# JzHuai0108/sim3opt

Measured on AMD Instinct MI355X. Metric: LM iterations/s, higher is better.
Workload: dtype f64

## Files before the change

sim3opt_amd/csrc/lm_kernels.hpp:

```cpp
#pragma once
__global__ __launch_bounds__(WG) void k_final_sum(const double* __restrict__ partials, int n,
                                                  double* __restrict__ out) {
  __shared__ double sh[4];
  const double s = sum_partials(partials, n, sh);
  if (threadIdx.x == 0) *out = s;
}

__global__ __launch_bounds__(WG) void k_final_trace_max(const double* __restrict__ trace_partials,
                                                        const double* __restrict__ max_partials, int n,
                                                        double* __restrict__ trace_out,
                                                        unsigned long long* __restrict__ maxdiag_bits) {
  __shared__ double sh[4];
  __shared__ double shm[4];
  const double s = sum_partials(trace_partials, n, sh);
  double m = 0.0;
  for (int i = threadIdx.x; i < n; i += WG) m = fmax(m, max_partials[i]);
#pragma unroll
  for (int off = 32; off > 0; off >>= 1) m = fmax(m, __shfl_xor(m, off));
  if ((threadIdx.x & 63) == 0) shm[threadIdx.x >> 6] = m;
  __syncthreads();
  if (threadIdx.x == 0) {
    *trace_out = s;
    m = fmax(fmax(shm[0], shm[1]), fmax(shm[2], shm[3]));
    *maxdiag_bits = (unsigned long long)__double_as_longlong(m);
  }
}

__global__ __launch_bounds__(WG) void k_final_sum_two(const double* __restrict__ pa, int na,
                                                      double* __restrict__ outa,
                                                      const double* __restrict__ pb, int nb_,
                                                      double* __restrict__ outb,
                                                      DevScalars* __restrict__ host_mirror,
                                                      const DevScalars* __restrict__ dev_sc) {
  __shared__ double sh[4];
  const double a = sum_partials(pa, na, sh);
  const double b = sum_partials(pb, nb_, sh);
  if (threadIdx.x == 0) {
    *outa = a;
    *outb = b;
    if (host_mirror) {
      host_mirror->chi2 = a;
      host_mirror->scale = b;
      host_mirror->fail = dev_sc->fail;
    }
  }
}

__device__ __forceinline__ double quad_form(const double e[7], const double* __restrict__ Om) {
  double acc = 0.0;
#pragma unroll
  for (int c = 0; c < 7; ++c) {
    double col = 0.0;
#pragma unroll
    for (int r = 0; r < 7; ++r) col += e[r] * Om[7 * c + r];
    acc += col * e[c];
  }
  return acc;
}

__device__ __forceinline__ void huber(double e2, double delta, double& rho, double& w) {
  const double dsqr = delta * delta;
  if (e2 <= dsqr) {
    rho = e2;
    w = 1.0;
  } else {
    const double sq = sqrt(e2);
    rho = 2 * sq * delta - dsqr;
    w = delta / sq;
  }
}


struct EdgeArgs {
  int32_t e_lo, e_hi;
  const int32_t* ev0;
  const int32_t* ev1;
  const Sim3* meas;
  const double* info;
  const double* kdelta;
  const Sim3* states;
  sim3::Opts opts;
};

__global__ __launch_bounds__(WG) void k_chi2(EdgeArgs A, double* __restrict__ partials) {
  __shared__ double sh[4];
  double acc = 0.0;
  for (int k = A.e_lo + blockIdx.x * WG + threadIdx.x; k < A.e_hi; k += gridDim.x * WG) {
    const Sim3 C = load_sim3(A.meas + k);
    const Sim3 S0 = load_sim3(A.states + A.ev0[k]);
    const Sim3 S1 = load_sim3(A.states + A.ev1[k]);
    double e[7];
    sim3::edge_error(C, S0, S1, A.opts, e);
    double chi;
    if (A.info) {
      chi = quad_form(e, A.info + (size_t)49 * k);
    } else {
      chi = 0.0;
#pragma unroll
      for (int r = 0; r < 7; ++r) chi += e[r] * e[r];
    }
    if (A.kdelta && A.kdelta[k] > 0.0) {
      double rho, w;
      huber(chi, A.kdelta[k], rho, w);
      chi = rho;
    }
    acc += chi;
  }
  const double s = block_sum(acc, sh);
  if (threadIdx.x == 0) partials[blockIdx.x] = s;
}

__global__ __launch_bounds__(WG) void k_edge_errors(EdgeArgs A, double* __restrict__ out) {
  for (int k = A.e_lo + blockIdx.x * WG + threadIdx.x; k < A.e_hi; k += gridDim.x * WG) {
    const Sim3 C = load_sim3(A.meas + k);
    const Sim3 S0 = load_sim3(A.states + A.ev0[k]);
    const Sim3 S1 = load_sim3(A.states + A.ev1[k]);
    double e[7];
    sim3::edge_error(C, S0, S1, A.opts, e);
#pragma unroll
    for (int r = 0; r < 7; ++r) out[(size_t)7 * k + r] = e[r];
  }
}

struct LinArgs {
  int32_t n_active;
  const int32_t* active;
  const int32_t* ev0;
  const int32_t* ev1;
  const Sim3* meas;
  const double* info;
  const double* kdelta;
  const Sim3* states;
  const int32_t* slot01;
  const int32_t* slot10;
  const int32_t* inc0;
  const int32_t* inc1;
  double* vals;
  double* scratch;
  double delta;
  sim3::Opts opts;
  const Sim3* ptab;
  int32_t dof_mask;
  DevScalars* sc;
};

struct GramTables {
  unsigned char ga[119], gb[119];
  unsigned char tr[28], tc[28];
};
__constant__ GramTables c_tab;

constexpr int EPB = 8;

__global__ __launch_bounds__(64) void k_perturbation_table(double delta, sim3::Opts opts, Sim3* __restrict__ tab) {
  const int t = threadIdx.x;
  if (t >= 14) return;
  const int d = t >> 1;
  const double step = (t & 1) ? -delta : delta;
  double xi[7];
#pragma unroll
  for (int i = 0; i < 7; ++i) xi[i] = (i == d) ? step : 0.0;
  tab[t] = sim3::exp(xi, opts);
}

template <bool HAS_INFO, bool HAS_KERNEL>
__device__ __forceinline__ void linearize_gram_store(const LinArgs& A, int edge, bool valid, int l,
                                                     double (*J)[7], double (*O)[7], double (*G)[15]) {
  __syncthreads();
  if (HAS_INFO) {
    if (valid) {
      const double* Om = A.info + (size_t)49 * edge;
      for (int t = l; t < 105; t += 32) {
        const int a = t / 7, r = t % 7;
        double acc = 0.0;
#pragma unroll
        for (int k = 0; k < 7; ++k) acc += Om[7 * k + r] * J[a][k];
        O[a][r] = acc;
      }
    }
    __syncthreads();
  }
  double (*OJ)[7] = HAS_INFO ? O : J;
  double w = 1.0;
  if (HAS_KERNEL) {
    if (valid && A.kdelta[edge] > 0.0) {
      double chi = 0.0, rho;
#pragma unroll
      for (int r = 0; r < 7; ++r) chi += J[14][r] * OJ[14][r];
      huber(chi, A.kdelta[edge], rho, w);
    }
  }
  if (valid) {
    for (int t = l; t < 119; t += 32) {
      const int a = c_tab.ga[t], b = c_tab.gb[t];
      double acc = 0.0;
#pragma unroll
      for (int r = 0; r < 7; ++r) acc += J[a][r] * OJ[b][r];
      G[a][b] = (b == 14 ? -w : w) * acc;
    }
  }
  __syncthreads();
  if (valid) {
    const int s01 = A.slot01[edge], s10 = A.slot10[edge];
    const int i0 = A.inc0[edge], i1 = A.inc1[edge];
    for (int o = l; o < 168; o += 32) {
      if (o < 49) {
        if (s01 >= 0) A.vals[(size_t)49 * s01 + o] = G[o % 7][7 + o / 7];
      } else if (o < 98) {
        const int p = o - 49;
        if (s10 >= 0) A.vals[(size_t)49 * s10 + p] = G[p / 7][7 + p % 7];
      } else if (o < 133) {
        const int t = o - 98;
        if (i0 >= 0)
          A.scratch[(size_t)35 * i0 + t] = t < 28 ? G[c_tab.tr[t]][c_tab.tc[t]] : G[t - 28][14];
      } else {
        const int t = o - 133;
        if (i1 >= 0)
          A.scratch[(size_t)35 * i1 + t] =
              t < 28 ? G[7 + c_tab.tr[t]][7 + c_tab.tc[t]] : G[7 + t - 28][14];
      }
    }
  }
}

template <bool HAS_INFO, bool HAS_KERNEL>
__global__ __launch_bounds__(WG) void k_linearize_numeric(LinArgs A) {
  __shared__ double s_in[EPB][24];
  __shared__ double s_J[EPB][15][7];
  __shared__ double s_O[HAS_INFO ? EPB : 1][15][7];
  __shared__ double s_G[EPB][14][15];
  const int l = threadIdx.x & 31, es = threadIdx.x >> 5;
  const int ai = blockIdx.x * EPB + es;
  const bool valid = ai < A.n_active;
  if (blockIdx.x == 0 && threadIdx.x == 0) A.sc->maxdiag_bits = 0ull;
  int edge = 0;
  if (valid) {
    edge = A.active[ai];
    if (l < 8) s_in[es][l] = reinterpret_cast<const double*>(A.meas + edge)[l];
    else if (l < 16) s_in[es][l] = reinterpret_cast<const double*>(A.states + A.ev0[edge])[l - 8];
    else if (l < 24) s_in[es][l] = reinterpret_cast<const double*>(A.states + A.ev1[edge])[l - 16];
  }
  __syncthreads();
  double e[7] = {0, 0, 0, 0, 0, 0, 0};
  if (valid && l < 29) {
    Sim3 C, S0, S1;
    const double* in = s_in[es];
    C.q[0] = in[0]; C.q[1] = in[1]; C.q[2] = in[2]; C.q[3] = in[3];
    C.t[0] = in[4]; C.t[1] = in[5]; C.t[2] = in[6]; C.s = in[7];
    S0.q[0] = in[8]; S0.q[1] = in[9]; S0.q[2] = in[10]; S0.q[3] = in[11];
    S0.t[0] = in[12]; S0.t[1] = in[13]; S0.t[2] = in[14]; S0.s = in[15];
    S1.q[0] = in[16]; S1.q[1] = in[17]; S1.q[2] = in[18]; S1.q[3] = in[19];
    S1.t[0] = in[20]; S1.t[1] = in[21]; S1.t[2] = in[22]; S1.s = in[23];
    if (l < 28) {
      const Sim3 P = A.ptab[l % 14];
      if (l < 14) S0 = sim3::mul(P, S0);
      else S1 = sim3::mul(P, S1);
    }
    sim3::edge_error(C, S0, S1, A.opts, e);
  }
  const double scalar = 1.0 / (2.0 * A.delta);
#pragma unroll
  for (int r = 0; r < 7; ++r) {
    const double other = __shfl_down(e[r], 1);
    if (valid && l < 28 && !(l & 1))
      s_J[es][l >> 1][r] = ((A.dof_mask >> ((l % 14) >> 1)) & 1) ? scalar * (e[r] - other) : 0.0;
    if (valid && l == 28) s_J[es][14][r] = e[r];
  }
  linearize_gram_store<HAS_INFO, HAS_KERNEL>(A, edge, valid, l, s_J[es], HAS_INFO ? s_O[es] : s_J[es], s_G[es]);
}

template <bool HAS_INFO, bool HAS_KERNEL>
__global__ __launch_bounds__(WG) void k_linearize_analytic(LinArgs A) {
  constexpr int NJ = EPB * 15 * 7, NO = HAS_INFO ? NJ : 7, NG = EPB * 14 * 15;
  constexpr int NS = sim3::JAC_SUMS + 13;
  constexpr int NN = EPB * (sim3::JAC_NODES + 1) * sim3::JAC_SUMS, NM = EPB * NS;
  constexpr int NLDS = NN + NM > NJ + NO + NG ? NN + NM : NJ + NO + NG;
  __shared__ double s_in[EPB][24];
  __shared__ double s_lds[NLDS];
  double (*s_node)[sim3::JAC_NODES + 1][sim3::JAC_SUMS] =
      reinterpret_cast<double (*)[sim3::JAC_NODES + 1][sim3::JAC_SUMS]>(s_lds);
  double (*s_M)[NS] = reinterpret_cast<double (*)[NS]>(s_lds + NN);
  double (*s_J)[15][7] = reinterpret_cast<double (*)[15][7]>(s_lds);
  double (*s_O)[15][7] = reinterpret_cast<double (*)[15][7]>(s_lds + NJ);
  double (*s_G)[14][15] = reinterpret_cast<double (*)[14][15]>(s_lds + NJ + NO);
  const int l = threadIdx.x & 31, es = threadIdx.x >> 5;
  const int ai = blockIdx.x * EPB + es;
  const bool valid = ai < A.n_active;
  if (blockIdx.x == 0 && threadIdx.x == 0) A.sc->maxdiag_bits = 0ull;
  int edge = 0;
  if (valid) {
    edge = A.active[ai];
    if (l < 8) s_in[es][l] = reinterpret_cast<const double*>(A.meas + edge)[l];
    else if (l < 16) s_in[es][l] = reinterpret_cast<const double*>(A.states + A.ev0[edge])[l - 8];
    else if (l < 24) s_in[es][l] = reinterpret_cast<const double*>(A.states + A.ev1[edge])[l - 16];
  }
  __syncthreads();
  double e[7] = {0, 0, 0, 0, 0, 0, 0};
  Sim3 C;
  if (valid) {
    Sim3 S0, S1;
    const double* in = s_in[es];
    C.q[0] = in[0]; C.q[1] = in[1]; C.q[2] = in[2]; C.q[3] = in[3];
    C.t[0] = in[4]; C.t[1] = in[5]; C.t[2] = in[6]; C.s = in[7];
    S0.q[0] = in[8]; S0.q[1] = in[9]; S0.q[2] = in[10]; S0.q[3] = in[11];
    S0.t[0] = in[12]; S0.t[1] = in[13]; S0.t[2] = in[14]; S0.s = in[15];
    S1.q[0] = in[16]; S1.q[1] = in[17]; S1.q[2] = in[18]; S1.q[3] = in[19];
    S1.t[0] = in[20]; S1.t[1] = in[21]; S1.t[2] = in[22]; S1.s = in[23];
    sim3::edge_error(C, S0, S1, A.opts, e);
    if (l < sim3::JAC_NODES) {
      double v[sim3::JAC_SUMS];
      sim3::left_jacobian_node(e, l, v);
#pragma unroll
      for (int i = 0; i < sim3::JAC_SUMS; ++i) s_node[es][l][i] = v[i];
    } else if (l == sim3::JAC_NODES) {
      double X[13];
      sim3::exp_of_residual(e, X);
#pragma unroll
      for (int i = 0; i < 13; ++i) s_node[es][l][i] = X[i];
    }
  }
  __syncthreads();
  if (valid && l < sim3::JAC_SUMS) {
    double acc = 0.0;
#pragma unroll
    for (int k = 0; k < sim3::JAC_NODES; ++k) acc += s_node[es][k][l];
    s_M[es][l] = acc;
    if (l < 13) s_M[es][sim3::JAC_SUMS + l] = s_node[es][sim3::JAC_NODES][l];
  }
  __syncthreads();
  if (valid && l < 15) {
    double col[7];
    if (l < 14) {
      sim3::edge_jacobian_column(s_M[es], s_M[es] + sim3::JAC_SUMS, C, l, A.dof_mask, col);
    } else {
#pragma unroll
      for (int r = 0; r < 7; ++r) col[r] = e[r];
    }
#pragma unroll
    for (int r = 0; r < 7; ++r) s_J[es][l][r] = col[r];
  }
  linearize_gram_store<HAS_INFO, HAS_KERNEL>(A, edge, valid, l, s_J[es], HAS_INFO ? s_O[es] : s_J[es], s_G[es]);
}

__global__ __launch_bounds__(WG) void k_edge_jacobians(EdgeArgs A, int dof_mask, double* __restrict__ e_out,
                                                      double* __restrict__ J_out) {
  for (int k = A.e_lo + blockIdx.x * WG + threadIdx.x; k < A.e_hi; k += gridDim.x * WG) {
    const Sim3 C = load_sim3(A.meas + k);
    const Sim3 S0 = load_sim3(A.states + A.ev0[k]);
    const Sim3 S1 = load_sim3(A.states + A.ev1[k]);
    double e[7], M[sim3::JAC_SUMS], X[13];
    sim3::edge_error(C, S0, S1, A.opts, e);
    sim3::left_jacobian_blocks(e, M);
    sim3::exp_of_residual(e, X);
#pragma unroll
    for (int r = 0; r < 7; ++r) e_out[(size_t)7 * k + r] = e[r];
    for (int c = 0; c < 14; ++c) {
      double col[7];
      sim3::edge_jacobian_column(M, X, C, c, dof_mask, col);
#pragma unroll
      for (int r = 0; r < 7; ++r) J_out[(size_t)98 * k + 14 * r + c] = col[r];
    }
  }
}

__global__ __launch_bounds__(WG) void k_diag_reduce(int r0, int r1,
                                                    const int32_t* __restrict__ incptr,
                                                    const int32_t* __restrict__ rowptr,
                                                    const double* __restrict__ scratch,
                                                    double* __restrict__ vals,
                                                    double* __restrict__ b, DevScalars* sc,
                                                    double* __restrict__ trace_partials,
                                                    double* __restrict__ max_partials) {
  __shared__ double sh[4];
  __shared__ double shm[4];
  const int lane = threadIdx.x & 63;
  const int wave = threadIdx.x >> 6;
  const int r = lane % 7, c = lane / 7;
  const int m = r < c ? r : c, M = r < c ? c : r;
  const int tsrc = lane < 49 ? (M * (M + 1)) / 2 + m : 0;
  const int bsrc = lane < 7 ? 28 + lane : 0;
  double dmax = 0.0, tr = 0.0;
  for (int row = r0 + blockIdx.x * 4 + wave; row < r1; row += gridDim.x * 4) {
    const int k0 = incptr[row], k1 = incptr[row + 1];
    double sum = 0.0;
    if (lane < 35)
      for (int k = k0; k < k1; ++k) sum += scratch[(size_t)35 * k + lane];
    const double v = __shfl(sum, tsrc);
    const double bv = __shfl(sum, bsrc);
    if (lane < 49) {
      vals[(size_t)49 * rowptr[row] + lane] = v;
      if (r == c) {
        dmax = fmax(dmax, fabs(v));
        tr += v;
      }
    }
    if (lane < 7) b[(size_t)7 * row + lane] = bv;
  }
#pragma unroll
  for (int off = 32; off > 0; off >>= 1) dmax = fmax(dmax, __shfl_xor(dmax, off));
  if (lane == 0) shm[wave] = dmax;
  const double ts = block_sum(tr, sh);
  if (threadIdx.x == 0) {
    trace_partials[blockIdx.x] = ts;
    max_partials[blockIdx.x] = fmax(fmax(shm[0], shm[1]), fmax(shm[2], shm[3]));
  }
}

__global__ __launch_bounds__(WG) void k_oplus(int nv, const int32_t* __restrict__ hidx,
                                              const double* __restrict__ x, Sim3* states,
                                              sim3::Opts opts, const DevScalars* sc, Sim3* backup,
                                              int fail_token) {
  const int v = blockIdx.x * WG + threadIdx.x;
  if (v >= nv) return;
  if (backup) {
    const double* s8 = reinterpret_cast<const double*>(states + v);
    double* b8 = reinterpret_cast<double*>(backup + v);
#pragma unroll
    for (int i = 0; i < 8; ++i) b8[i] = s8[i];
  }
  if (sc && sc->fail == fail_token) return;
  const int h = hidx[v];
  if (h < 0) return;
  double xi[7];
#pragma unroll
  for (int i = 0; i < 7; ++i) xi[i] = x[(size_t)7 * h + i];
  const Sim3 P = sim3::exp(xi, opts);
  const Sim3 S = sim3::mul(P, load_sim3(states + v));
  double* d = reinterpret_cast<double*>(states + v);
  d[0] = S.q[0]; d[1] = S.q[1]; d[2] = S.q[2]; d[3] = S.q[3];
  d[4] = S.t[0]; d[5] = S.t[1]; d[6] = S.t[2]; d[7] = S.s;
}

__global__ __launch_bounds__(WG) void k_copy_states(int nv, const Sim3* __restrict__ src, Sim3* __restrict__ dst) {
  const int i = blockIdx.x * WG + threadIdx.x;
  if (i < 8 * nv) reinterpret_cast<double*>(dst)[i] = reinterpret_cast<const double*>(src)[i];
}

__global__ __launch_bounds__(WG) void k_scale(int j0, int j1, const double* __restrict__ x,
                                              const double* __restrict__ b, double lambda,
                                              double* __restrict__ partials) {
  __shared__ double sh[4];
  double acc = 0.0;
  for (int j = j0 + blockIdx.x * WG + threadIdx.x; j < j1; j += gridDim.x * WG)
    acc += x[j] * (lambda * x[j] + b[j]);
  const double s = block_sum(acc, sh);
  if (threadIdx.x == 0) partials[blockIdx.x] = s;
}

__global__ __launch_bounds__(WG) void k_count_unpoisoned(const uint32_t* __restrict__ p, size_t nwords,
                                                         unsigned long long* __restrict__ count) {
  unsigned long long c = 0;
  for (size_t i = (size_t)blockIdx.x * WG + threadIdx.x; i < nwords; i += (size_t)gridDim.x * WG)
    c += p[i] != 0xFFFFFFFFu;
  if (c) atomicAdd(count, c);
}
```

Measured before the change: 47.46.

## Use wave-local LDS sync in numeric linearize and batch scratch reduction loads

In the numeric linearization kernel, block-wide barriers are replaced with wave-local LDS syncs, since each 32-lane edge group only touches its own shared slices. The Gram and store loops are unrolled with fixed trip counts, and the perturbed state is rebuilt from shared memory before the multiply instead of branching on which state gets replaced. The diagonal-block accumulation loads eight scratch entries at a time with nontemporal loads to raise memory-level parallelism. If two 32-lane groups share one 64-wide wave, wave-local sync is sufficient, but this relies on lockstep semantics and adds register pressure.

After: 48.32 (median of 6 runs). +1.8%, better.

```diff
diff --git a/sim3opt_amd/csrc/lm_kernels.hpp b/sim3opt_amd/csrc/lm_kernels.hpp
--- a/sim3opt_amd/csrc/lm_kernels.hpp
+++ b/sim3opt_amd/csrc/lm_kernels.hpp
@@ -163,14 +163,23 @@
   tab[t] = sim3::exp(xi, opts);
 }
 
-template <bool HAS_INFO, bool HAS_KERNEL>
+template <bool WAVE_LOCAL>
+__device__ __forceinline__ void lin_sync() {
+  if (WAVE_LOCAL) wave_lds_sync();
+  else __syncthreads();
+}
+
+template <bool HAS_INFO, bool HAS_KERNEL, bool WAVE_LOCAL>
 __device__ __forceinline__ void linearize_gram_store(const LinArgs& A, int edge, bool valid, int l,
                                                      double (*J)[7], double (*O)[7], double (*G)[15]) {
-  __syncthreads();
+  lin_sync<WAVE_LOCAL>();
   if (HAS_INFO) {
     if (valid) {
       const double* Om = A.info + (size_t)49 * edge;
-      for (int t = l; t < 105; t += 32) {
+#pragma unroll
+      for (int i = 0; i < 4; ++i) {
+        const int t = l + 32 * i;
+        if (t >= 105) break;
         const int a = t / 7, r = t % 7;
         double acc = 0.0;
 #pragma unroll
@@ -178,7 +187,7 @@
         O[a][r] = acc;
       }
     }
-    __syncthreads();
+    lin_sync<WAVE_LOCAL>();
   }
   double (*OJ)[7] = HAS_INFO ? O : J;
   double w = 1.0;
@@ -191,7 +200,10 @@
     }
   }
   if (valid) {
-    for (int t = l; t < 119; t += 32) {
+#pragma unroll
+    for (int i = 0; i < 4; ++i) {
+      const int t = l + 32 * i;
+      if (t >= 119) break;
       const int a = c_tab.ga[t], b = c_tab.gb[t];
       double acc = 0.0;
 #pragma unroll
@@ -199,11 +211,14 @@
       G[a][b] = (b == 14 ? -w : w) * acc;
     }
   }
-  __syncthreads();
+  lin_sync<WAVE_LOCAL>();
   if (valid) {
     const int s01 = A.slot01[edge], s10 = A.slot10[edge];
     const int i0 = A.inc0[edge], i1 = A.inc1[edge];
-    for (int o = l; o < 168; o += 32) {
+#pragma unroll
+    for (int i = 0; i < 6; ++i) {
+      const int o = l + 32 * i;
+      if (o >= 168) break;
       if (o < 49) {
         if (s01 >= 0) A.vals[(size_t)49 * s01 + o] = G[o % 7][7 + o / 7];
       } else if (o < 98) {
@@ -240,7 +255,7 @@
     else if (l < 16) s_in[es][l] = reinterpret_cast<const double*>(A.states + A.ev0[edge])[l - 8];
     else if (l < 24) s_in[es][l] = reinterpret_cast<const double*>(A.states + A.ev1[edge])[l - 16];
   }
-  __syncthreads();
+  wave_lds_sync();
   double e[7] = {0, 0, 0, 0, 0, 0, 0};
   if (valid && l < 29) {
     Sim3 C, S0, S1;
@@ -253,8 +268,14 @@
     S1.t[0] = in[20]; S1.t[1] = in[21]; S1.t[2] = in[22]; S1.s = in[23];
     if (l < 28) {
       const Sim3 P = A.ptab[l % 14];
-      if (l < 14) S0 = sim3::mul(P, S0);
-      else S1 = sim3::mul(P, S1);
+      const bool first = l < 14;
+      const double* x = in + (first ? 8 : 16);
+      Sim3 X;
+      X.q[0] = x[0]; X.q[1] = x[1]; X.q[2] = x[2]; X.q[3] = x[3];
+      X.t[0] = x[4]; X.t[1] = x[5]; X.t[2] = x[6]; X.s = x[7];
+      const Sim3 Q = sim3::mul(P, X);
+      if (first) S0 = Q;
+      else S1 = Q;
     }
     sim3::edge_error(C, S0, S1, A.opts, e);
   }
@@ -266,7 +287,7 @@
       s_J[es][l >> 1][r] = ((A.dof_mask >> ((l % 14) >> 1)) & 1) ? scalar * (e[r] - other) : 0.0;
     if (valid && l == 28) s_J[es][14][r] = e[r];
   }
-  linearize_gram_store<HAS_INFO, HAS_KERNEL>(A, edge, valid, l, s_J[es], HAS_INFO ? s_O[es] : s_J[es], s_G[es]);
+  linearize_gram_store<HAS_INFO, HAS_KERNEL, true>(A, edge, valid, l, s_J[es], HAS_INFO ? s_O[es] : s_J[es], s_G[es]);
 }
 
 template <bool HAS_INFO, bool HAS_KERNEL>
@@ -339,7 +360,7 @@
 #pragma unroll
     for (int r = 0; r < 7; ++r) s_J[es][l][r] = col[r];
   }
-  linearize_gram_store<HAS_INFO, HAS_KERNEL>(A, edge, valid, l, s_J[es], HAS_INFO ? s_O[es] : s_J[es], s_G[es]);
+  linearize_gram_store<HAS_INFO, HAS_KERNEL, false>(A, edge, valid, l, s_J[es], HAS_INFO ? s_O[es] : s_J[es], s_G[es]);
 }
 
 __global__ __launch_bounds__(WG) void k_edge_jacobians(EdgeArgs A, int dof_mask, double* __restrict__ e_out,
@@ -383,8 +404,26 @@
   for (int row = r0 + blockIdx.x * 4 + wave; row < r1; row += gridDim.x * 4) {
     const int k0 = incptr[row], k1 = incptr[row + 1];
     double sum = 0.0;
-    if (lane < 35)
-      for (int k = k0; k < k1; ++k) sum += scratch[(size_t)35 * k + lane];
+    if (lane < 35) {
+      const double* p = scratch + (size_t)35 * k0 + lane;
+      int n = k1 - k0;
+      for (; n >= 8; n -= 8, p += 8 * 35) {
+        double x[8];
+#pragma unroll
+        for (int j = 0; j < 8; ++j) x[j] = __builtin_nontemporal_load(p + 35 * j);
+#pragma unroll
+        for (int j = 0; j < 8; ++j) sum += x[j];
+      }
+      if (n > 0) {
+        double x[7];
+#pragma unroll
+        for (int j = 0; j < 7; ++j)
+          if (j < n) x[j] = __builtin_nontemporal_load(p + 35 * j);
+#pragma unroll
+        for (int j = 0; j < 7; ++j)
+          if (j < n) sum += x[j];
+      }
+    }
     const double v = __shfl(sum, tsrc);
     const double bv = __shfl(sum, bsrc);
     if (lane < 49) {
```
